# 1mishra/cbc

Hardware: AMD Instinct MI355X
Metric: Mbases/s encoded (bit-exact) on synthetic 150 bp SAM (higher is better)
Workload: dtype u32; 1 GPU; cfg2: synthetic 150 bp SAM, 10000000 reads per GPU vs a 248956422 bp uniform-ACGT contig, block-parallel encode; reads_rank0=10000000, blocks_rank0=2442, block_reads=4096, lds_bytes_per_block=15264, payload_bytes_rank0=20710203, parallelism=one GPU, no collective

## Files before the change

cbc_amd/csrc/cbc_encode_body.h:

```cpp
#ifndef CBC_ENCODE_BODY_H
#define CBC_ENCODE_BODY_H

#include <stdint.h>
#include <type_traits>
#include "../../include/cbc_gpu.h"
#include "cbc_plan.h"

#ifndef CBC_PRIO_CODER
#define CBC_PRIO_CODER 3
#define CBC_PRIO_MODEL 0
#endif
#define CBC_REC_PACK_AT 56u
#define CBC_AWORD     26u
#define CBC_M26       ((1u << 26) - 1u)
#define CBC_M25       ((1u << 25) - 1u)
#define CBC_RESCALE   (1u << 20)
#define CBC_NVARCTX   0xffffu
#define CBC_NOMEMO    0xffffffffu
#define CBC_BLOOM_LOG2 13u
#define CBC_ROLE_FUSED 0u
#define CBC_ROLE_MODEL 1u
#define CBC_ROLE_CODER 2u

#define CBC_LT_MATCH   0u
#define CBC_LT_SAMEREF 8u
#define CBC_LT_CHARS   16u

#define CBC_LDS_RLEN    0u
#define CBC_LDS_SNPS    256u
#define CBC_LDS_INDELS  512u
#define CBC_LDS_RNKEY   768u
#define CBC_LDS_RNEXC   (768u + CBC_CAP_NAME)
#define CBC_LDS_BLOOM   (768u + 2u * CBC_CAP_NAME)
#define CBC_LDS_P0      (768u + 2u * CBC_CAP_NAME + CBC_BLOOM_WORDS)
#define CBC_LDS_BATCH   CBC_PLAN_TABLE_WORDS
#ifndef CBC_BATCH_MIN
#define CBC_BATCH_MIN   40u
#endif
#define CBC_LDS_CTL     (CBC_LDS_BATCH + CBC_BATCH_SLOTS * CBC_BATCH_WORDS)
#define CBC_LDS_RING    (CBC_LDS_CTL + 8u)
#define CBC_LDS_RUN     (CBC_LDS_RING + CBC_RING_WORDS)
#define CBC_LDS_FIXED   CBC_PLAN_LDS_FIXED_WORDS

#ifdef CBC_EMU_TRACE
extern "C" void cbc_emu_trace(uint32_t read, uint32_t lo, uint32_t cnt, uint32_t n);
#endif

struct cbc_enc_args {
    const cbc_read_rec   *recs;
    const uint8_t        *seq;
    const uint32_t       *tok;
    const uint8_t        *names;
    const cbc_block_desc *blocks;
    const uint8_t        *ref;
    uint8_t              *out;
    cbc_block_result     *results;
    uint64_t ref_bytes, out_bytes, seq_bytes, n_tok, n_recs;
    uint32_t n_blocks, cap_pos, cap_var, names_bytes;
};

#if defined(CBC_STAMP) && defined(__HIP_DEVICE_COMPILE__)
#define CBC_T0() do { unsigned long long t_; asm volatile("s_memtime %0\n\ts_waitcnt lgkmcnt(0)" : "=s"(t_) :: "memory"); E.t_last = t_; } while (0)
#define CBC_TS(k) do { unsigned long long t_; asm volatile("s_memtime %0\n\ts_waitcnt lgkmcnt(0)" : "=s"(t_) :: "memory"); E.t_sum[k] += t_ - E.t_last; E.t_last = t_; } while (0)
#define CBC_TSM(k) do { unsigned long long t_; asm volatile("s_memtime %0\n\ts_waitcnt lgkmcnt(0)" : "=s"(t_) :: "memory"); t_sum[k] += t_ - t_last; t_last = t_; } while (0)
#elif defined(CBC_MARKS) && defined(__HIP_DEVICE_COMPILE__)
#define CBC_TSM(k) asm volatile("; ==== CBC_MARK M" #k)
#define CBC_T0() asm volatile("; ==== CBC_MARK start")
#define CBC_TS(k) asm volatile("; ==== CBC_MARK " #k)
#else
#define CBC_T0() do {} while (0)
#define CBC_TS(k) do {} while (0)
#define CBC_TSM(k) do {} while (0)
#endif

CBC_FN bool cbc_le64(uint64_t a, uint64_t b)
{
    uint32_t ah = (uint32_t)(a >> 32), al = (uint32_t)a, bh = (uint32_t)(b >> 32), bl = (uint32_t)b;
    return (ah < bh) | ((ah == bh) & (al <= bl));
}
CBC_FN bool cbc_fits64(uint64_t off, uint64_t len, uint64_t total)
{
    return cbc_le64(off, total) && cbc_le64(len, total - off);
}
CBC_FN uint32_t cbc_avail32(uint64_t total, uint32_t off)
{
    uint64_t a = total - off;
    if (!cbc_le64((uint64_t)off, total)) return 0u;
    return (uint32_t)(a >> 32) ? 0xffffffffu : (uint32_t)a;
}
CBC_FN uint32_t cbc_basepair(uint32_t c)
{
    return c == 'A' ? 0u : c == 'C' ? 1u : c == 'G' ? 2u : c == 'T' ? 3u : 4u;
}
// ... 76 lines not shown
        w2 |= (kw == 2u) ? bit : 0ull;
        w3 |= (kw == 3u) ? bit : 0ull;
    }
#endif
};

template <class W, class = void> struct CbcHasLaneN : std::false_type {};
template <class W> struct CbcHasLaneN<W, std::void_t<decltype(&W::set_lane2_uv), decltype(&W::set_lane3)>> : std::true_type {};

template <class W, bool GEN = false>
struct CbcEnc {
    typedef typename W::V32 V32;
    typedef typename W::Mask Mask;

    typedef typename W::Uv Uv;
    Uv l, rng;
    Uv lm1;
    Uv thr0;
    CBC_MFN void set_l_forms()
    {
        lm1 = W::uv_opaque(l - 1u);
        thr0 = ((l & (1u << 24)) | (1u << 25)) - l;
    }
    uint32_t scale3;
    uint32_t bitpos, flushed;
    uint32_t *ring;
    uint32_t *out32; uint32_t cap_words;
    uint32_t status, nsym, fail_read, cur_read;
    V32 q_lo, q_cnt, q_n; uint32_t q_len;
    uint32_t role, batch_i; uint32_t *batch, *ctl;
    V32 b_lo, b_hi, b_n, b_fl, b_fh; uint32_t b_len, b_pos, b_stop, b_flags, seen_last; uint64_t b_neq;
    V32 rec_a, rec_s; uint32_t rec_n;
#ifdef CBC_STAMP
    unsigned long long t_last, t_sum[16];
#endif

    V32 small;
    V32 fkey, fexc; uint32_t fcount;
    V32 hkey, hexc; uint32_t hc0, hc1, hc2, hc3, hn0, hn1, hn2, hn3;
    uint32_t *rlen_exc, *snps_exc, *indels_exc, *rname_key, *rname_exc, *pos_val, *pos_occ, *pos_pre, *pos_idx, *var_ev, *bloom, *p0ev;
    uint32_t *runs;
    uint32_t snps_n, indels_n;
    uint32_t rn_count, rn_cap;
    uint32_t *vtab;
    uint32_t *fsp_key, *fsp_exc; uint32_t fsp_count;
    uint32_t *pos_ov_val, *pos_ov_occ; uint32_t pos_lds_cap;
    uint32_t *palpha; uint32_t pa_n0, pa_n1, pa_n2, pa_n3;
    uint32_t pos_card, cap_pos;
    uint32_t nev, nev1, cap_var;
    V32 p0cnt; uint32_t p0over;
    uint32_t L0;

    uint32_t prevPos, prevM, prevChar, win_pos;
    CbcWin<W> win;

    CBC_MFN void fail(uint32_t st) { if (status == CBC_ST_OK) { status = st; fail_read = cur_read; } }

    CBC_MFN void place(const V32 &val, const V32 &len, const V32 &off, const Mask &m)
    {
        const V32 aligned = val << (W::splat(32u) - len);
        const V32 sh = off & 31u, w = (off >> 5) & (CBC_RING_WORDS - 1u);
        const Mask on = m & (len != 0u);
        W::lds_or(ring, w, aligned >> sh, on);
        W::lds_or(ring, (w + 1u) & (CBC_RING_WORDS - 1u), aligned << (W::splat(32u) - sh), on & (sh != 0u));
    }
    CBC_MFN void flush_full()
    {
// ... 80 lines not shown
        else {
            V32 ln = W::lane();
            Mask here = ln == q_len;
            q_lo = W::select(here, W::splat(lo), q_lo);
            q_cnt = W::select(here, W::splat(cnt), q_cnt);
            q_n = W::select(here, W::splat(n), q_n);
        }
        q_len++;
    }
    CBC_MFN void rec_put(Uv rec, Uv k3)
    {
        if constexpr (!GEN && CbcHasLaneN<W>::value) W::set_lane2_uv(rec_a, rec_s, rec_n, rec, k3);
        else { W::set_lane_uv(rec_a, rec_n, rec); W::set_lane_uv(rec_s, rec_n, k3); }
    }
#define CBC_FRAC(c, n) W::frac32(c, n)
#define CBC_BF_LAST  1u
#define CBC_BF_GROUP 2u
#define CBC_END_N    0xffffffffu
    CBC_MFN void drain() { if (role == CBC_ROLE_MODEL) publish(0u, 0ull); else drain_q(); }
    CBC_MFN void seg_end()
    {
        if (role != CBC_ROLE_MODEL) { drain_q(); return; }
        if (q_len >= 64u) publish(0u, 0ull);
        q_put(0u, 1u, CBC_END_N);
    }
    CBC_MFN void seg_end_fits()
    {
        W::expect_eq(q_len < 64u ? 1u : 0u, 1u, "seg_end_fits: queue full");
        q_put(0u, 1u, CBC_END_N);
    }
    CBC_MFN void publish(uint32_t flags, uint64_t neq)
    {
        V32 ln = W::lane();
        CBC_TSM(5);
        while (batch_i - W::ctl_load(ctl + 1) >= CBC_BATCH_SLOTS) W::nap();
        CBC_TSM(6);
        uint32_t *buf = batch + (batch_i & (CBC_BATCH_SLOTS - 1u)) * CBC_BATCH_WORDS;
        Mask m = ln < q_len;
        W::store32(buf, ln, q_lo, m); W::store32(buf + 64u, ln, q_cnt, m); W::store32(buf + 128u, ln, q_n, m);
        V32 hdr = W::select(ln == 0u, W::splat(q_len), W::select(ln == 1u, W::splat(flags),
                  W::select(ln == 2u, W::splat(status), W::select(ln == 3u, W::splat(status == CBC_ST_OK ? cur_read : fail_read),
                  W::select(ln == 4u, W::splat((uint32_t)neq), W::splat((uint32_t)(neq >> 32)))))));
        W::store32(buf + 192u, ln, hdr, ln < 6u);
        batch_i++;
        W::ctl_store(ctl, batch_i);
        q_len = 0;
    }
    CBC_MFN void step(uint32_t lo, uint32_t hi, uint32_t n, uint32_t flo, uint32_t fhi)
    {
        Uv rec, k3;
        code1(lo, hi, n, flo, fhi, rec, k3);
        rec_put(rec, k3);
        nsym++;
        if (++rec_n >= CBC_REC_PACK_AT) { pack(rec_a, rec_s, rec_n); rec_n = 0; }
    }
    CBC_MFN void flush_recs() { if (rec_n) { pack(rec_a, rec_s, rec_n); rec_n = 0; } }
    CBC_MFN void room(uint32_t k) { if (rec_n + k >= 64u) flush_recs(); }
    template <class FLO, class FHI, class FN>
    CBC_MFN void step_fixed(FLO lo_of, FHI hi_of, FN n_of, uint32_t flo, uint32_t fhi)
    {
        Uv rec, k3;
        code1_lazy(flo, fhi, lo_of, hi_of, n_of, rec, k3);
#ifdef CBC_ABLATE_SETLANE
        rec_a ^= rec; rec_s ^= k3;
#else
        rec_put(rec, k3);
#endif
        nsym++; rec_n++;
    }
    template <class FLO, class FHI, class FN>
    CBC_MFN void step_fixed_quiet(FLO lo_of, FHI hi_of, FN n_of, uint32_t flo, uint32_t fhi)
    {
#ifdef CBC_ABLATE_CODER
        step_fixed(lo_of, hi_of, n_of, flo, fhi); return;
#endif
        Uv ql, qh, tl, th;
        W::mul64(rng, flo, ql, tl); W::mul64(rng, fhi, qh, th);
        if (W::uv_ge(tl | th, 0xfc000000u)) {
            const uint32_t lo = lo_of(), hi = hi_of(), n = n_of();
            ql += (rng * lo - ql * n >= n) ? 1u : 0u;
// ... 8 lines not shown
        if (W::uv_ge(still & (1u << 25), 1u)) {
#ifndef __HIP_DEVICE_COMPILE__
            const uint32_t lf = W::uv_scalar(l1), uf = W::uv_scalar(u);
            W::expect_eq(W::clz32((((lf ^ uf) & CBC_M26) << 6) | 32u), 0u, "step_fixed_quiet: E1/E2 would shift");
            W::expect_eq(W::clz32(((((~lf | uf) << 7) | 127u))), 0u, "step_fixed_quiet: E3 would shift");
#endif
            l = l1; rng = qh - ql;
            set_l_forms();
            nsym++;
            return;
        }
        Uv rec, k3;
        code_tail(ql, qh, rec, k3);
        rec_put(rec, k3);
        nsym++; rec_n++;
    }
    CBC_MFN void drain_q()
    {
        V32 ln = W::lane();
        uint32_t m = W::uni(q_len);
        const uint64_t bad = W::ballot((ln < m) & ((q_cnt == 0u) | (q_n == 0u)));
        if (bad) m = W::ctz64(bad);
        const V32 q_hi = q_lo + q_cnt;
        const V32 f_lo = CBC_FRAC(q_lo, q_n), f_hi = CBC_FRAC(q_hi, q_n);
        for (uint32_t k = 0; k < m; k++)
            step(W::readlane(q_lo, k), W::readlane(q_hi, k), W::readlane(q_n, k), W::readlane(f_lo, k), W::readlane(f_hi, k));
        if (bad) fail(CBC_ST_ASSERT);
        q_len = 0;
    }
    CBC_MFN void pull()
    {
        V32 ln = W::lane();
        CBC_TSM(9);
        while (W::ctl_load(ctl) == batch_i) W::nap();
        CBC_TSM(10);
        const uint32_t *buf = batch + (batch_i & (CBC_BATCH_SLOTS - 1u)) * CBC_BATCH_WORDS;
        V32 hdr = W::load32(buf + 192u, ln, ln < 6u, 0u);
        const uint32_t len = W::readlane(hdr, 0u);
        const uint32_t pst = W::readlane(hdr, 2u), prec = W::readlane(hdr, 3u);
        b_flags = W::readlane(hdr, 1u);
        b_neq = (uint64_t)W::readlane(hdr, 4u) | ((uint64_t)W::readlane(hdr, 5u) << 32);
        Mask m = ln < len;
        b_lo = W::load32(buf, ln, m, 0u); b_n = W::load32(buf + 128u, ln, m, 1u);
        const V32 cnt = W::load32(buf + 64u, ln, m, 1u);
        b_hi = b_lo + cnt;
        b_fl = CBC_FRAC(b_lo, b_n); b_fh = CBC_FRAC(b_hi, b_n);
        b_len = len > 64u ? 64u : len; b_pos = 0;
        const uint64_t bad = W::ballot(m & ((cnt == 0u) | (b_n == 0u)));
        b_stop = bad ? W::ctz64(bad) : 64u;
        batch_i++;
        W::ctl_store(ctl + 1, batch_i);
        if (b_flags & CBC_BF_LAST) seen_last = 1u;
        if (pst != CBC_ST_OK && status == CBC_ST_OK) { status = pst; fail_read = prec; }
    }
    CBC_MFN void seg_consume()
    {
        const V32 ln = W::lane();
        uint32_t done = 0u;
        while ((done | status) == 0u) {
            if (b_pos == b_len) {
                if (seen_last) fail(CBC_ST_ASSERT);
                else { pull(); if (b_flags & CBC_BF_GROUP) fail(CBC_ST_ASSERT); }
            } else {
                const uint64_t em = W::ballot((b_n == CBC_END_N) & (ln >= b_pos) & (ln < b_len));
                uint32_t kend = em ? W::ctz64(em) : b_len;
                const uint32_t bad = b_stop < kend ? 1u : 0u;
                if (bad) kend = b_stop;
                for (uint32_t k = b_pos; k < kend; k++) {
                    Uv rec, k3;
                    code1_lazy(W::readlane(b_fl, k), W::readlane(b_fh, k), [&]() -> uint32_t { return W::readlane(b_lo, k); },
                               [&]() -> uint32_t { return W::readlane(b_hi, k); }, [&]() -> uint32_t { return W::readlane(b_n, k); }, rec, k3);
                    rec_put(rec, k3);
                    nsym++;
                    if (++rec_n >= CBC_REC_PACK_AT) { pack(rec_a, rec_s, rec_n); rec_n = 0; }
                }
                if (bad) fail(CBC_ST_ASSERT);
                else if (em) { b_pos = kend + 1u; done = 1u; }
                else b_pos = kend;
            }
        }
    }
    CBC_MFN void consume_all()
    {
        while (!seen_last) {
            pull();
            if (status != CBC_ST_OK) continue;
            const uint32_t kend = b_stop < b_len ? b_stop : b_len;
            for (uint32_t k = 0; k < kend; k++) {
                Uv rec, k3;
                code1_lazy(W::readlane(b_fl, k), W::readlane(b_fh, k), [&]() -> uint32_t { return W::readlane(b_lo, k); },
                           [&]() -> uint32_t { return W::readlane(b_hi, k); }, [&]() -> uint32_t { return W::readlane(b_n, k); }, rec, k3);
                rec_put(rec, k3);
                nsym++;
                if (++rec_n >= CBC_REC_PACK_AT) { pack(rec_a, rec_s, rec_n); rec_n = 0; }
            }
            if (b_stop < b_len) fail(CBC_ST_ASSERT);
        }
    }
    CBC_MFN void post_group(uint32_t g, uint64_t neq, uint32_t refused)
    {
        W::write_uni(ctl, 4u + 2u * (g & 1u), (uint32_t)neq);
        W::write_uni(ctl, 5u + 2u * (g & 1u), (uint32_t)(neq >> 32));
        if (refused) W::write_uni(ctl, 3u, 1u);
        W::ctl_store(ctl + 2, g + 1u);
    }
    CBC_MFN void abort_groups()
    {
        W::write_uni(ctl, 3u, 1u);
        W::ctl_store(ctl + 2, 0xffffffffu);
    }
    CBC_MFN bool wait_group(uint32_t g, uint64_t &neq)
    {
        CBC_TSM(5);
        while (W::ctl_load(ctl + 2) < g + 1u) W::nap();
        CBC_TSM(6);
        neq = (uint64_t)W::read_uni(ctl, 4u + 2u * (g & 1u)) | ((uint64_t)W::read_uni(ctl, 5u + 2u * (g & 1u)) << 32);
        return W::read_uni(ctl, 3u) == 0u;
    }
    CBC_MFN uint64_t pull_group()
    {
        if (status != CBC_ST_OK) return 0ull;
        if (b_pos != b_len || seen_last) { fail(CBC_ST_ASSERT); return 0ull; }
        pull();
        if (status == CBC_ST_OK && !(b_flags & CBC_BF_GROUP)) fail(CBC_ST_ASSERT);
        return b_neq;
    }
    CBC_MFN void pull_rest() { while (!seen_last) pull(); }
    CBC_MFN void code1(uint32_t lo, uint32_t hi, uint32_t n, uint32_t flo, uint32_t fhi, Uv &rec, Uv &k3)
    {
        code1_lazy(flo, fhi, [&]() { return lo; }, [&]() { return hi; }, [&]() { return n; }, rec, k3);
    }
    template <class FLO, class FHI, class FN>
    CBC_MFN void code1_lazy(uint32_t flo, uint32_t fhi, FLO lo_of, FHI hi_of, FN n_of, Uv &rec, Uv &k3)
    {
#ifdef CBC_ABLATE_CODER
        l ^= flo; rng ^= fhi; rec = W::uv(0u); k3 = rec; return;
#endif
        const Uv range = rng;
        Uv ql, qh, tl, th;
        W::mul64(range, flo, ql, tl); W::mul64(range, fhi, qh, th);
        if (W::uv_ge(tl | th, 0xfc000000u)) {
            const uint32_t lo = lo_of(), hi = hi_of(), n = n_of();
            ql += (range * lo - ql * n >= n) ? 1u : 0u;
            qh += (range * hi - qh * n >= n) ? 1u : 0u;
        }
#ifndef __HIP_DEVICE_COMPILE__
        W::expect_eq(W::uv_scalar(ql), (uint32_t)((uint64_t)W::uv_scalar(range) * lo_of() / n_of()), "scaled_div(cum)");
        W::expect_eq(W::uv_scalar(qh), (uint32_t)((uint64_t)W::uv_scalar(range) * hi_of() / n_of()), "scaled_div(cum + count)");
#endif
        code_tail(ql, qh, rec, k3);
// ... 865 lines not shown
                }
            }
            CBC_TSM(13);
#undef CBC_SNP
#undef CBC_TOK
#undef CBC_READ_BYTE
    }
};

template <class W, uint32_t ROLE>
CBC_FN void cbc_encode_stream(const cbc_enc_args &A, uint32_t blk, uint32_t *lds)
{
    const uint32_t role = ROLE;
    typedef typename W::V32 V32;
    typedef typename W::Mask Mask;
    const V32 ln = W::lane();
    const cbc_block_desc *bd = A.blocks + blk;
    CbcEnc<W> E;

    const uint64_t rec_base = bd->rec_base, seq_base = bd->seq_base, tok_base = bd->tok_base;
    const uint64_t ref_off = bd->ref_off, out_off = bd->out_off;
    const uint32_t out_cap = bd->out_cap, n_reads = bd->n_reads, name_off = bd->name_off;
    const uint32_t L0 = bd->read_length, n_tok_blk = bd->n_tok;

    E.status = CBC_ST_OK; E.nsym = 0; E.fail_read = 0; E.cur_read = 0;
    E.l = W::uv(0u); E.set_l_forms(); E.rng = W::uv(CBC_M26 + 1u); E.scale3 = 0u; E.bitpos = 0; E.flushed = 0;
    E.ring = lds + CBC_LDS_RING;
    E.q_lo = W::splat(0u); E.q_cnt = W::splat(0u); E.q_n = W::splat(0u); E.q_len = 0;
    E.b_lo = W::splat(0u); E.b_hi = W::splat(0u); E.b_n = W::splat(1u); E.b_fl = W::splat(0u); E.b_fh = W::splat(0u);
    E.b_len = 0; E.b_pos = 0; E.b_stop = 64u; E.b_flags = 0; E.seen_last = 0; E.b_neq = 0;
    E.rec_a = W::splat(0u); E.rec_s = W::splat(0u); E.rec_n = 0;
    E.role = role; E.batch_i = 0; E.batch = lds + CBC_LDS_BATCH; E.ctl = lds + CBC_LDS_CTL;
    if (ROLE != CBC_ROLE_FUSED) {
        if (ROLE == CBC_ROLE_MODEL) { W::write_uni(E.ctl, 0u, 0u); W::write_uni(E.ctl, 1u, 0u); W::write_uni(E.ctl, 2u, 0u); W::write_uni(E.ctl, 3u, 0u); }
        W::barrier();
    }
    const uint32_t payload_cap = bd->reserved;
    E.out32 = (uint32_t *)(A.out + out_off);
    E.cap_words = payload_cap >> 2;
    E.var_ev = (uint32_t *)(A.out + out_off + payload_cap);
    E.cap_var = payload_cap <= out_cap ? (out_cap - payload_cap) >> 2 : 0u;
    bool args_ok = cbc_fits64(out_off, out_cap, A.out_bytes) && ((out_off & 3u) == 0) && ((payload_cap & 3u) == 0) &&
                   (payload_cap <= out_cap) &&
                   cbc_fits64(rec_base, n_reads, A.n_recs) && cbc_fits64(tok_base, n_tok_blk, A.n_tok) &&
                   (L0 >= 1u && L0 <= 256u) && (name_off < A.names_bytes);
    if (!args_ok) { E.cap_words = 0; E.fail(CBC_ST_ASSERT); }
    if (n_reads > CBC_MAX_BLOCK_READS) E.fail(CBC_ST_UNSUPPORTED);

    E.L0 = L0;
    E.rlen_exc = lds + CBC_LDS_RLEN; E.snps_exc = lds + CBC_LDS_SNPS; E.indels_exc = lds + CBC_LDS_INDELS;
    E.rname_key = lds + CBC_LDS_RNKEY; E.rname_exc = lds + CBC_LDS_RNEXC;
    E.bloom = lds + CBC_LDS_BLOOM; E.p0ev = lds + CBC_LDS_P0; E.runs = lds + CBC_LDS_RUN;
    E.pos_val = lds + CBC_LDS_FIXED; E.pos_occ = E.pos_val + A.cap_pos; E.pos_pre = E.pos_occ + A.cap_pos;
    E.fsp_key = E.fsp_exc = nullptr; E.fsp_count = 0; E.pos_ov_val = E.pos_ov_occ = nullptr; E.pos_lds_cap = 0xffffffc0u; E.palpha = nullptr;
    E.pos_idx = E.pos_pre + A.cap_pos;
    E.cap_pos = A.cap_pos;
    if (ROLE != CBC_ROLE_MODEL) {
        for (uint32_t b = 0; b < CBC_POS_IDX_WORDS; b += 64u) W::store32(E.pos_idx, ln + b, W::splat(0u), W::all());
        for (uint32_t b = 0; b < CBC_RING_WORDS; b += 64u) W::store32(E.ring, ln + b, W::splat(0u), W::all());
        for (uint32_t b = 0; b < 256u; b += 64u) W::store32(E.rlen_exc, ln + b, W::splat(0u), W::all());
        W::write_uni(E.pos_val, 0u, 0xffffffffu); W::write_uni(E.pos_occ, 0u, 0u); W::write_uni(E.pos_pre, 0u, 0u);
    }
    if (ROLE != CBC_ROLE_CODER) {
        for (uint32_t b = 0; b < 512u; b += 64u) W::store32(E.snps_exc, ln + b, W::splat(0u), W::all());
        for (uint32_t b = 0; b < CBC_BLOOM_WORDS; b += 64u) W::store32(E.bloom, ln + b, W::splat(0u), W::all());
    }
    E.p0cnt = W::splat(0u); E.p0over = 0;
    E.snps_n = L0; E.indels_n = L0;
    E.rn_count = 0; E.rn_cap = CBC_CAP_NAME; E.vtab = nullptr;
    E.pos_card = 1u;
    E.nev = 0; E.nev1 = 0;
    E.fkey = W::splat(0u); E.fexc = W::splat(0u); E.fcount = 0;
    E.hkey = W::splat(0u); E.hexc = W::splat(0u);
    E.hc0 = E.hc1 = E.hc2 = E.hc3 = 0; E.hn0 = E.hn1 = E.hn2 = E.hn3 = 256u;
    {
        V32 sm = W::splat(0u);
        sm = W::select(ln < 10u, W::splat(1u), sm);
        V32 r = (ln - CBC_LT_CHARS) >> 3, c = (ln - CBC_LT_CHARS) & 7u;
        Mask inch = (ln >= CBC_LT_CHARS) & (r < 6u) & (c < 5u);
        V32 cv = W::select(c == 4u, W::splat(1u), W::select(c == r, W::splat(0u), W::splat(8u)));
        Mask bump = ((r == 0u) & ((c == 1u) | (c == 2u))) | ((r == 1u) & ((c == 0u) | (c == 3u))) |
                    ((r == 2u) & ((c == 0u) | (c == 3u))) | ((r == 3u) & ((c == 1u) | (c == 2u)));
        cv = W::select(bump, cv + 8u, cv);
        sm = W::select(inch, cv, sm);
        E.small = sm;
    }
    E.prevPos = 0; E.prevM = 0; E.prevChar = 0; E.win_pos = 0;
    E.win_clear();

    const uint4 *recs4 = (const uint4 *)(A.recs + rec_base);
    const uint8_t *seqb = A.seq + seq_base;
    const uint32_t *tokb = A.tok + tok_base;
    const uint8_t *refb = A.ref + ref_off;
    const uint64_t seq_avail = cbc_le64(seq_base, A.seq_bytes) ? A.seq_bytes - seq_base : 0;
    const uint64_t ref_avail = cbc_le64(ref_off, A.ref_bytes) ? A.ref_bytes - ref_off : 0;
    const uint32_t seq_lim = cbc_avail32(seq_avail, 0u), ref_lim = cbc_avail32(ref_avail, 0u);
#ifdef CBC_STAMP
    for (int i = 0; i < 16; i++) E.t_sum[i] = 0;
    CBC_T0();
#endif

    auto gen_header = [&]() {
        for (uint32_t k = 0; k < 34u && E.status == CBC_ST_OK; k++) {
            uint32_t v = (k == 0u) ? L0 : (k == 33u) ? 8u : CBC_WELL_SEED;
            E.regsparse_code(E.hkey, E.hexc, 0u, 8u, E.hc0, E.hn0, 256u, 1u, v >> 24, CBC_ST_ASSERT);
            E.regsparse_code(E.hkey, E.hexc, 8u, 8u, E.hc1, E.hn1, 256u, 1u, (v >> 16) & 0xffu, CBC_ST_ASSERT);
            E.regsparse_code(E.hkey, E.hexc, 16u, 8u, E.hc2, E.hn2, 256u, 1u, (v >> 8) & 0xffu, CBC_ST_ASSERT);
            E.regsparse_code(E.hkey, E.hexc, 24u, 8u, E.hc3, E.hn3, 256u, 1u, v & 0xffu, CBC_ST_ASSERT);
            if ((k & 7u) == 7u) E.drain();
        }
    };
    auto gen_rname = [&]() {
        for (uint32_t q = 0; E.status == CBC_ST_OK; q++) {
            uint32_t ch = (name_off + q < A.names_bytes) ? W::read_uni8(A.names, name_off + q) : 0u;
            E.rname_code(E.prevChar, ch);
            if ((q & 31u) == 31u) E.drain();
            if (ch == 0u) break;
            E.prevChar = ch;
        }
    };
    auto gen_sentinel = [&]() {
        if (E.q_len >= 56u) E.drain();
        E.cur_read = n_reads;
        E.rname_code(E.prevChar, (uint32_t)'\n');
        E.rname_code((uint32_t)'\n', 0u);
    };
    auto match_group = [&](uint32_t cn, const V32 &r_pos, const V32 &r_fl, const V32 &r_seq) -> uint64_t {
        const V32 vrl = W::select(ln < cn, r_fl >> 16, W::splat(0u));
        const V32 ro = r_pos - 1u;
        const uint32_t nd = W::uni(W::readlane(W::scan_incl_max(vrl), 63u) >> 2);
        V32 acc = W::splat(0u);
// ... 50 lines not shown
            if (c0 == 0u) { gen_rname(); E.seg_end(); }
            typename CbcEnc<W>::Prep P;
            E.prep_group(P, neq, r_tok, tokb, n_tok_blk);
            CBC_TS(14);
            uint64_t todo = neq;
            V32 nx_seq = W::splat(0u), nx_tok = W::splat(0u);
            uint32_t nx_j = 64u;
            auto prefetch = [&](uint32_t jn) {
                const uint32_t so = W::readlane(r_seq, jn), to = W::readlane(r_tok, jn), nrl = W::readlane(r_fl, jn) >> 16;
                V32 bo = ln * 4u;
                nx_seq = W::load32_bytes(seqb + so, bo, bo < nrl);
                nx_tok = W::load32(tokb + to, ln, (ln + to) < n_tok_blk, 0u);
                nx_j = jn;
            };
            auto prefetch_if_general = [&](uint64_t rest) {
                if (rest) { const uint32_t jn = W::ctz64(rest); if (!((P.ord >> jn) & 1ull)) prefetch(jn); }
            };
            typename CbcEnc<W>::Run R;
            R.pk = W::splat(0u); R.ca = R.pk; R.cb = R.pk; R.rm = 0ull; R.s = 0u; R.counted = 0u;
            while (todo && E.status == CBC_ST_OK) {
                const uint32_t j = W::ctz64(todo);
                if ((P.ord >> j) & 1ull) {
                    if (!E.run_pass(R, P, todo, r_pos, r_fl, r_seq, r_tok, tokb, seqb)) { P.ord &= ~R.rm; continue; }
                    todo &= ~R.rm;
                    prefetch_if_general(todo);
                    CBC_TS(2);
                    for (uint64_t rr = R.rm; rr && E.status == CBC_ST_OK; rr &= rr - 1ull) {
                        const uint32_t jr = W::ctz64(rr);
                        E.cur_read = c0 + jr;
                        E.run_record(R, W::readlane(P.hdr0, jr) >> 16, W::readlane(P.lo, jr), W::readlane(P.cnt, jr));
                        E.seg_end_fits();
                        CBC_TS(1);
                        if (E.q_len >= CBC_BATCH_MIN) E.drain();
                    }
                    continue;
                }
                if (nx_j != j) prefetch(j);
                todo &= todo - 1ull;
                E.cur_read = c0 + j;
                const V32 seqv = nx_seq, tokv = nx_tok;
                prefetch_if_general(todo);
                const typename CbcEnc<W>::PrepRec pr = { W::readlane(P.lo, j), W::readlane(P.cnt, j) };
                E.edits(W::readlane(r_pos, j), W::readlane(r_fl, j), W::readlane(r_tok, j), seqv, tokv, tokb, n_tok_blk, pr);
                E.seg_end_fits();
                CBC_TS(1);
                if (E.q_len >= CBC_BATCH_MIN) E.drain();
            }
        }
        if (E.status == CBC_ST_OK) { gen_sentinel(); E.seg_end(); }
#if defined(CBC_STAMP) && defined(__HIP_DEVICE_COMPILE__)
        if (E.cap_var >= 64u) for (int i = 0; i < 16; i++) {
            W::write_uni(E.var_ev + E.cap_var - 32u, 2 * i, (uint32_t)E.t_sum[i]); W::write_uni(E.var_ev + E.cap_var - 32u, 2 * i + 1, (uint32_t)(E.t_sum[i] >> 32)); }
#endif
        E.publish(CBC_BF_LAST, 0ull);
        return;
    }

    const bool fused = ROLE == CBC_ROLE_FUSED;
    if (!fused) W::prio(CBC_PRIO_CODER);
#ifndef CBC_MATCH_IN_MODEL
    uint64_t neq_ahead = 0;
    auto look_ahead = [&](uint32_t g0) {
        V32 a_pos, a_fl, a_seq, a_tok;
        const uint32_t an = n_reads - g0 < 64u ? n_reads - g0 : 64u;
        const uint32_t saved = E.cur_read;
        CBC_TS(9);
        const bool okg = load_group(g0, a_pos, a_fl, a_seq, a_tok, true);
        neq_ahead = okg ? match_group(an, a_pos, a_fl, a_seq) : 0ull;
        E.post_group(g0 >> 6, neq_ahead, okg ? 0u : 1u);
        CBC_TS(15);
        if (okg) E.cur_read = saved;
    };
    if (!fused && n_reads != 0u && E.status == CBC_ST_OK) look_ahead(0u);
#endif
    if (E.status == CBC_ST_OK) { if (fused) { gen_header(); E.seg_end(); } else E.seg_consume(); }
    for (uint32_t c0 = 0; c0 < n_reads && E.status == CBC_ST_OK; c0 += 64u) {
        V32 r_pos, r_fl, r_seq, r_tok;
        const uint32_t cn = n_reads - c0 < 64u ? n_reads - c0 : 64u;
        E.cur_read = c0;
        uint64_t neq;
        typename CbcEnc<W>::Prep P;
        typename CbcEnc<W>::Run R;
        R.pk = W::splat(0u); R.ca = R.pk; R.cb = R.pk; R.rm = 0ull; R.s = 0u; R.counted = 0u;
        if (fused) {
            if (!load_group(c0, r_pos, r_fl, r_seq, r_tok, true)) break;
            neq = match_group(cn, r_pos, r_fl, r_seq);
// ... 79 lines not shown
        typedef std::integral_constant<int, 0> Plain; typedef std::integral_constant<int, 1> Esc; typedef std::integral_constant<int, 2> Look;
        uint32_t j = 0;
        if (c0 == 0u && jn != 0u) { code_record(0u, std::true_type(), Look()); j = 1u; }
        while (j < jn && E.status == CBC_ST_OK) {
            const uint64_t ahead = F.esc >> j;
            uint32_t run_end = ahead ? j + W::ctz64(ahead) : jn;
            if (run_end > jn) run_end = jn;
            for (; j < run_end && E.status == CBC_ST_OK; j++) code_record(j, std::false_type(), Plain());
            if (j < jn && E.status == CBC_ST_OK) { code_record(j, std::false_type(), Esc()); j++; }
        }
#else
        for (uint32_t j = 0; j < jn && E.status == CBC_ST_OK; j++) code_record(j, 0, std::integral_constant<int, 2>());
#endif
#undef CBC_ENC_FIRST
        if (jn < cn && E.status == CBC_ST_OK) { E.cur_read = c0 + jn; E.fail(W::readlane(F.st, jn)); }
    }
    uint32_t nbytes = 0;
    if (E.status == CBC_ST_OK) {
        E.cur_read = n_reads;
        if (n_reads) E.encode(10u * n_reads - 9u, 11u, 10u * n_reads + 2u);
        else E.encode(1u, 1u, 2u);
        E.drain_q();
        if (fused) { gen_sentinel(); E.seg_end(); } else E.seg_consume();
    }
    if (E.status == CBC_ST_OK) { E.flush_recs(); nbytes = E.finish(); }
    if (E.status != CBC_ST_OK) nbytes = 0;
#ifndef CBC_MATCH_IN_MODEL
#ifndef CBC_MATCH_NO_ABORT_FOR_TEST
    if (!fused && E.status != CBC_ST_OK) E.abort_groups();
#endif
#endif
    if (!fused) E.pull_rest();
#if defined(CBC_STAMP) && defined(__HIP_DEVICE_COMPILE__)
    if (payload_cap >= 128u) for (int i = 0; i < 16; i++) {
        W::write_uni(E.out32, 2 * i, (uint32_t)E.t_sum[i]); W::write_uni(E.out32, 2 * i + 1, (uint32_t)(E.t_sum[i] >> 32)); }
#endif
    V32 resv = W::select(ln == 0u, W::splat(nbytes), W::select(ln == 1u, W::splat(E.status),
               W::select(ln == 2u, W::splat(E.nsym), W::splat(E.fail_read))));
    W::store32((uint32_t *)(A.results + blk), ln, resv, ln < 4u);
}

#endif
```

cbc_amd/csrc/cbc_long_body.h:

```cpp
#ifndef CBC_LONG_BODY_H
#define CBC_LONG_BODY_H

#include "cbc_encode_body.h"
#include "cbc_decode_body.h"

#define CBC_LONG_MAGIC 0x43424C03u
#define CBC_LLDS_GAPLO  0u
#define CBC_LLDS_SP     512u
#define CBC_LLDS_RNKEY  896u
#define CBC_LLDS_RNEXC  (896u + CBC_CAP_NAME)
#define CBC_LLDS_ROLE   (896u + 2u * CBC_CAP_NAME)
#define CBC_LLDS_RING   CBC_LLDS_ROLE
#define CBC_LLDS_BATCH  (CBC_LLDS_ROLE + CBC_RING_WORDS)
#define CBC_LLDS_CTL    (CBC_LLDS_BATCH + CBC_BATCH_SLOTS * CBC_BATCH_WORDS)

#define CBC_LLDS_TRIP   (CBC_LLDS_CTL + 8u)
#define CBC_LLDS_FIXED  (CBC_LLDS_TRIP + 576u)
static inline uint32_t cbc_long_lds_bytes(uint32_t cap_pos) { return 4u * (CBC_LLDS_FIXED + 2u * cap_pos); }
static inline uint32_t cbc_long_dec_lds_bytes(uint32_t cap_pos) { return 4u * (CBC_LLDS_ROLE + 2u * cap_pos); }
#define CBC_LSCR_GAPHI  0u
#define CBC_LSCR_GX     1536u
#define CBC_LSCR_EDITS  2048u
#ifndef CBC_LONG_EDIT_CAP
#define CBC_LONG_EDIT_CAP 8192u
#endif
#define CBC_LONG_EDIT_HALF (CBC_LONG_EDIT_CAP / 2u)
#define CBC_LONG_TABLE_WORDS 2048u
#define CBC_ROLE_WALKER 3u
#define CBC_LONG_SCRATCH_WORDS (2048u + CBC_LONG_EDIT_CAP)

#define CBC_LS_LEN 0u
#define CBC_LS_NE  4u
CBC_FN uint32_t cbc_long_kind_base(uint32_t pk) { return pk < 2u ? pk * 3u : 10u + (pk - 2u) * 3u; }

struct cbc_long_args {
    const cbc_read_rec   *recs;
    const uint8_t        *seq;
    const uint32_t       *tok;
    const uint8_t        *names;
    const cbc_block_desc *blocks;
    const uint8_t        *ref;
    uint8_t              *out;
    cbc_block_result     *results;
    uint64_t ref_bytes, out_bytes, seq_bytes, n_tok, n_recs;
    uint32_t n_blocks, cap_pos, names_bytes;
    uint32_t *scratch;
};
// ... 29 lines not shown
};

template <class W, uint32_t ROLE>
CBC_FN void cbc_long_encode(const cbc_long_args &A, uint32_t blk, uint32_t *lds)
{
    typedef typename W::V32 V32;
    typedef typename W::Mask Mask;
    typedef CbcEnc<W, true> Enc;
    const V32 ln = W::lane();
    const cbc_block_desc *bd = A.blocks + blk;
    Enc E;
    const uint64_t rec_base = bd->rec_base, seq_base = bd->seq_base, tok_base = bd->tok_base, ref_off = bd->ref_off, out_off = bd->out_off;
    const uint32_t out_cap = bd->out_cap, n_reads = bd->n_reads, name_off = bd->name_off, n_tok_blk = bd->n_tok;

    E.status = CBC_ST_OK; E.nsym = 0; E.fail_read = 0; E.cur_read = 0;
    E.l = W::uv(0u); E.set_l_forms(); E.rng = W::uv(CBC_M26 + 1u); E.scale3 = 0u; E.bitpos = 0; E.flushed = 0;
    E.ring = lds + CBC_LLDS_RING;
    E.q_lo = W::splat(0u); E.q_cnt = W::splat(0u); E.q_n = W::splat(0u); E.q_len = 0;
    E.b_lo = W::splat(0u); E.b_hi = W::splat(0u); E.b_n = W::splat(1u); E.b_fl = W::splat(0u); E.b_fh = W::splat(0u);
    E.rec_a = W::splat(0u); E.rec_s = W::splat(0u); E.rec_n = 0;
    E.role = ROLE; E.batch_i = 0; E.batch = lds + CBC_LLDS_BATCH; E.ctl = lds + CBC_LLDS_CTL;
    E.b_len = 0; E.b_pos = 0; E.b_stop = 64u; E.b_flags = 0; E.seen_last = 0; E.b_neq = 0;
    if (ROLE != CBC_ROLE_FUSED) {
        if (ROLE == CBC_ROLE_MODEL) for (uint32_t k = 0; k < 8u; k++) W::write_uni(E.ctl, k, 0u);
        W::barrier();
    }
    E.out32 = (uint32_t *)(A.out + out_off);
    E.cap_words = out_cap >> 2;
    bool args_ok = cbc_fits64(out_off, out_cap, A.out_bytes) && ((out_off & 3u) == 0u) && cbc_fits64(rec_base, n_reads, A.n_recs) &&
                   cbc_fits64(tok_base, n_tok_blk, A.n_tok) && (name_off < A.names_bytes) && A.cap_pos >= 2u && n_reads <= 64u &&
                   A.scratch != nullptr;
    if (!args_ok) { E.cap_words = 0; E.fail(CBC_ST_ASSERT); }
#ifdef CBC_STAMP
    for (int i = 0; i < 16; i++) E.t_sum[i] = 0;
    CBC_T0();
#endif

    if (ROLE == CBC_ROLE_CODER) {
        W::prio(CBC_PRIO_CODER);
        for (uint32_t b = 0; b < CBC_RING_WORDS; b += 64u) W::store32(E.ring, ln + b, W::splat(0u), W::all());
        E.consume_all();
        uint32_t nbytes = 0;
        if (E.status == CBC_ST_OK) { E.flush_recs(); nbytes = E.finish(); }
        if (E.status != CBC_ST_OK) nbytes = 0;
#if defined(CBC_STAMP) && defined(__HIP_DEVICE_COMPILE__)
        CBC_TS(9);
        if (out_cap >= 512u) for (int i = 0; i < 16; i++) {
            W::write_uni(E.out32, 2 * i, (uint32_t)E.t_sum[i]); W::write_uni(E.out32, 2 * i + 1, (uint32_t)(E.t_sum[i] >> 32)); }
#endif
        V32 resv = W::select(ln == 0u, W::splat(nbytes), W::select(ln == 1u, W::splat(E.status),
                   W::select(ln == 2u, W::splat(E.nsym), W::splat(E.fail_read))));
        W::store32((uint32_t *)(A.results + blk), ln, resv, ln < 4u);
        return;
    }

    E.L0 = 256u;
    E.rlen_exc = nullptr; E.snps_exc = nullptr; E.indels_exc = nullptr;
    E.rname_key = lds + CBC_LLDS_RNKEY; E.rname_exc = lds + CBC_LLDS_RNEXC; E.rn_cap = CBC_CAP_NAME; E.rn_count = 0;
    E.pos_val = lds + CBC_LLDS_FIXED; E.pos_occ = E.pos_val + A.cap_pos; E.pos_pre = nullptr; E.cap_pos = A.cap_pos;
    E.fsp_key = E.fsp_exc = nullptr; E.fsp_count = 0; E.pos_ov_val = E.pos_ov_occ = nullptr; E.pos_lds_cap = 0xffffffc0u; E.palpha = nullptr;
    E.bloom = nullptr; E.var_ev = nullptr; E.nev = E.nev1 = 0; E.cap_var = 0; E.vtab = nullptr; E.p0ev = nullptr;
    E.p0cnt = W::splat(0u); E.p0over = 0;
    uint32_t *scr = A.scratch + (uint64_t)blk * CBC_LONG_SCRATCH_WORDS;
    if (ROLE != CBC_ROLE_WALKER) {
        for (uint32_t b = 0; b < CBC_LLDS_SP; b += 64u) W::store32(lds, ln + b, W::splat(0u), W::all());
        if (E.status == CBC_ST_OK) for (uint32_t b = 0; b < CBC_LONG_TABLE_WORDS; b += 64u) W::store32_list(scr, ln + b, W::splat(0u), W::all());
        if (ROLE == CBC_ROLE_FUSED) for (uint32_t b = 0; b < CBC_RING_WORDS; b += 64u) W::store32(E.ring, ln + b, W::splat(0u), W::all());
// ... 740 lines not shown
```

cbc_amd/csrc/cbc_plan.h:

```cpp
#ifndef CBC_PLAN_H
#define CBC_PLAN_H

#include <stdint.h>
#include <string.h>
#include "../../include/cbc_gpu.h"

#define CBC_BLOOM_WORDS 256u
#define CBC_P0_WORDS    512u
#define CBC_P0_BUCKET_WORDS 64u
#define CBC_P0_CAP      128u
#define CBC_PLAN_TABLE_WORDS (768u + 2u * CBC_CAP_NAME + CBC_BLOOM_WORDS + 2u * CBC_P0_WORDS)
#ifndef CBC_BATCH_SLOTS
#define CBC_BATCH_SLOTS 2u
#endif
#define CBC_BATCH_WORDS 200u
#ifndef CBC_POS_IDX_WORDS
#define CBC_POS_IDX_WORDS 256u
#endif
#define CBC_RING_WORDS  256u
#define CBC_RUN_WORDS   16u
#define CBC_PLAN_LDS_FIXED_WORDS (CBC_PLAN_TABLE_WORDS + CBC_BATCH_SLOTS * CBC_BATCH_WORDS + 8u + CBC_RING_WORDS + CBC_RUN_WORDS)

static inline uint32_t cbc_plan_lds_bytes(const cbc_lds_caps *caps)
{
    return 4u * (CBC_PLAN_LDS_FIXED_WORDS + 3u * caps->cap_pos + CBC_POS_IDX_WORDS);
}

#define CBC_PLAN_DLDS_SCRATCH_WORDS 336u
#define CBC_PLAN_DLDS_FIXED_WORDS (CBC_PLAN_TABLE_WORDS + CBC_PLAN_DLDS_SCRATCH_WORDS + 768u)
static inline uint32_t cbc_plan_dec_lds_bytes(const cbc_lds_caps *caps)
{
    return 4u * (CBC_PLAN_DLDS_FIXED_WORDS + 2u * caps->cap_pos);
}

static inline uint64_t cbc_plan_block_area(cbc_block_desc *bd, uint64_t off, uint64_t nev)
{
    const uint64_t nsym = 136u + 2u * CBC_CAP_NAME + 16ull * bd->n_reads + 2 * nev;
    uint64_t payload_cap = (3 * nsym + 256 + 255) & ~255ull;
    uint64_t cap = payload_cap + ((4 * (nev + 64) + 255) & ~255ull);
    if (cap > 0xffffff00ull) { cap = 0xffffff00ull; payload_cap = cap / 2; payload_cap &= ~255ull; }
    bd->out_off = off; bd->out_cap = (uint32_t)cap; bd->reserved = (uint32_t)payload_cap;
    return cap;
}

static inline uint64_t cbc_plan_output(cbc_block_desc *blocks, uint32_t n_blocks,
                                       const cbc_read_rec *recs, const uint32_t *tok)
{
    uint64_t off = 0;
    for (uint32_t b = 0; b < n_blocks; b++) {
        cbc_block_desc *bd = &blocks[b];
        uint64_t nev = 0;
        for (uint32_t r = 0; r < bd->n_reads; r++) {
            const cbc_read_rec *rr = &recs[bd->rec_base + r];
            const uint32_t *t = tok + bd->tok_base + rr->tok_off;
// ... 75 lines not shown
```

Before: 235,300 Mbases/s.

## Parameterize model-coder hand-off ring and add acked multi-slot group masks

```diff
diff --git a/cbc_amd/csrc/cbc_encode_body.h b/cbc_amd/csrc/cbc_encode_body.h
--- a/cbc_amd/csrc/cbc_encode_body.h
+++ b/cbc_amd/csrc/cbc_encode_body.h
@@ -35,10 +35,16 @@
 #define CBC_LDS_P0      (768u + 2u * CBC_CAP_NAME + CBC_BLOOM_WORDS)
 #define CBC_LDS_BATCH   CBC_PLAN_TABLE_WORDS
 #ifndef CBC_BATCH_MIN
-#define CBC_BATCH_MIN   40u
-#endif
-#define CBC_LDS_CTL     (CBC_LDS_BATCH + CBC_BATCH_SLOTS * CBC_BATCH_WORDS)
-#define CBC_LDS_RING    (CBC_LDS_CTL + 8u)
+#define CBC_BATCH_MIN   (5u * CBC_BATCH_ENTRIES / 8u)
+#endif
+#define CBC_LDS_CTL     (CBC_LDS_BATCH + CBC_BATCH_SLOTS * CBC_BATCH_SLOT_WORDS)
+#define CBC_LDS_RING    (CBC_LDS_CTL + CBC_CTL_WORDS)
+#define CBC_CTL_PRODUCED 0u
+#define CBC_CTL_CONSUMED 1u
+#define CBC_CTL_POSTED   2u
+#define CBC_CTL_REFUSED  3u
+#define CBC_CTL_ACKED    4u
+#define CBC_CTL_MASKS    5u
 #define CBC_LDS_RUN     (CBC_LDS_RING + CBC_RING_WORDS)
 #define CBC_LDS_FIXED   CBC_PLAN_LDS_FIXED_WORDS
 
@@ -59,6 +65,7 @@
     uint32_t n_blocks, cap_pos, cap_var, names_bytes;
 };
 
+#define CBC_STAMP_SLOTS 20
 #if defined(CBC_STAMP) && defined(__HIP_DEVICE_COMPILE__)
 #define CBC_T0() do { unsigned long long t_; asm volatile("s_memtime %0\n\ts_waitcnt lgkmcnt(0)" : "=s"(t_) :: "memory"); E.t_last = t_; } while (0)
 #define CBC_TS(k) do { unsigned long long t_; asm volatile("s_memtime %0\n\ts_waitcnt lgkmcnt(0)" : "=s"(t_) :: "memory"); E.t_sum[k] += t_ - E.t_last; E.t_last = t_; } while (0)
@@ -201,7 +208,7 @@
     V32 b_lo, b_hi, b_n, b_fl, b_fh; uint32_t b_len, b_pos, b_stop, b_flags, seen_last; uint64_t b_neq;
     V32 rec_a, rec_s; uint32_t rec_n;
 #ifdef CBC_STAMP
-    unsigned long long t_last, t_sum[16];
+    unsigned long long t_last, t_sum[CBC_STAMP_SLOTS];
 #endif
 
     V32 small;
@@ -348,20 +355,54 @@
     CBC_MFN void publish(uint32_t flags, uint64_t neq)
     {
         V32 ln = W::lane();
-        CBC_TSM(5);
-        while (batch_i - W::ctl_load(ctl + 1) >= CBC_BATCH_SLOTS) W::nap();
-        CBC_TSM(6);
-        uint32_t *buf = batch + (batch_i & (CBC_BATCH_SLOTS - 1u)) * CBC_BATCH_WORDS;
-        Mask m = ln < q_len;
-        W::store32(buf, ln, q_lo, m); W::store32(buf + 64u, ln, q_cnt, m); W::store32(buf + 128u, ln, q_n, m);
-        V32 hdr = W::select(ln == 0u, W::splat(q_len), W::select(ln == 1u, W::splat(flags),
-                  W::select(ln == 2u, W::splat(status), W::select(ln == 3u, W::splat(status == CBC_ST_OK ? cur_read : fail_read),
-                  W::select(ln == 4u, W::splat((uint32_t)neq), W::splat((uint32_t)(neq >> 32)))))));
-        W::store32(buf + 192u, ln, hdr, ln < 6u);
-        batch_i++;
-        W::ctl_store(ctl, batch_i);
-        q_len = 0;
-    }
+        if constexpr (GEN) {
+            CBC_TSM(5);
+#ifdef CBC_STAMP
+            t_sum[18] += 1u; if (batch_i - W::ctl_load(ctl + 1) >= CBC_LONG_BATCH_SLOTS) t_sum[17] += 1u;
+#endif
+            while (batch_i - W::ctl_load(ctl + 1) >= CBC_LONG_BATCH_SLOTS) W::nap();
+            CBC_TSM(6);
+            uint32_t *buf = batch + (batch_i & (CBC_LONG_BATCH_SLOTS - 1u)) * CBC_LONG_BATCH_WORDS;
+            Mask m = ln < q_len;
+            W::store32(buf, ln, q_lo, m); W::store32(buf + 64u, ln, q_cnt, m); W::store32(buf + 128u, ln, q_n, m);
+            V32 hdr = W::select(ln == 0u, W::splat(q_len), W::select(ln == 1u, W::splat(flags),
+                      W::select(ln == 2u, W::splat(status), W::select(ln == 3u, W::splat(status == CBC_ST_OK ? cur_read : fail_read),
+                      W::select(ln == 4u, W::splat((uint32_t)neq), W::splat((uint32_t)(neq >> 32)))))));
+            W::store32(buf + 192u, ln, hdr, ln < 6u);
+            batch_i++;
+            W::ctl_store(ctl, batch_i);
+            q_len = 0;
+        } else {
+            uint32_t off = 0u;
+            do {
+                const uint32_t left = q_len - off;
+                const uint32_t n = CBC_BATCH_ENTRIES >= 64u || left < CBC_BATCH_ENTRIES ? left : CBC_BATCH_ENTRIES;
+                const uint32_t fl = n == left ? flags : 0u;
+                CBC_TSM(5);
+#ifdef CBC_STAMP
+                t_sum[18] += 1u; if (batch_i - W::ctl_load(ctl + CBC_CTL_CONSUMED) >= CBC_BATCH_SLOTS) t_sum[17] += 1u;
+#endif
+                while (batch_i - W::ctl_load(ctl + CBC_CTL_CONSUMED) >= CBC_BATCH_SLOTS) W::nap();
+                CBC_TSM(6);
+                uint32_t *buf = batch + (batch_i % CBC_BATCH_SLOTS) * CBC_BATCH_SLOT_WORDS;
+                const V32 k = ln - off;
+                const Mask m = k < n;
+                W::store32(buf, k, q_lo, m); W::store32(buf + CBC_BATCH_ENTRIES, k, q_cnt, m); W::store32(buf + 2u * CBC_BATCH_ENTRIES, k, q_n, m);
+#ifdef CBC_MATCH_IN_MODEL
+                if (fl & CBC_BF_GROUP) { W::write_uni(buf, 0u, (uint32_t)neq); W::write_uni(buf, 1u, (uint32_t)(neq >> 32)); }
+#endif
+                const V32 hdr = W::select(ln == 0u, W::splat(n | (fl << 8) | (status << 16)), W::splat(status == CBC_ST_OK ? cur_read : fail_read));
+                W::store32(buf + 3u * CBC_BATCH_ENTRIES, ln, hdr, ln < 2u);
+                batch_i++;
+                W::ctl_store(ctl + CBC_CTL_PRODUCED, batch_i);
+                off += n;
+            } while (CBC_BATCH_ENTRIES < 64u && off < q_len);
+            q_len = 0;
+        }
+    }
+#ifdef CBC_HANDOFF_ADAPTIVE
+    CBC_MFN bool coder_near() { return batch_i - W::ctl_load(ctl + CBC_CTL_CONSUMED) <= 1u; }
+#endif
     CBC_MFN void step(uint32_t lo, uint32_t hi, uint32_t n, uint32_t flo, uint32_t fhi)
     {
         Uv rec, k3;
@@ -436,26 +477,52 @@
     {
         V32 ln = W::lane();
         CBC_TSM(9);
+#ifdef CBC_STAMP
+        t_sum[18] += 1u; if (W::ctl_load(ctl) == batch_i) t_sum[17] += 1u;
+#endif
         while (W::ctl_load(ctl) == batch_i) W::nap();
         CBC_TSM(10);
-        const uint32_t *buf = batch + (batch_i & (CBC_BATCH_SLOTS - 1u)) * CBC_BATCH_WORDS;
-        V32 hdr = W::load32(buf + 192u, ln, ln < 6u, 0u);
-        const uint32_t len = W::readlane(hdr, 0u);
-        const uint32_t pst = W::readlane(hdr, 2u), prec = W::readlane(hdr, 3u);
-        b_flags = W::readlane(hdr, 1u);
-        b_neq = (uint64_t)W::readlane(hdr, 4u) | ((uint64_t)W::readlane(hdr, 5u) << 32);
-        Mask m = ln < len;
-        b_lo = W::load32(buf, ln, m, 0u); b_n = W::load32(buf + 128u, ln, m, 1u);
-        const V32 cnt = W::load32(buf + 64u, ln, m, 1u);
-        b_hi = b_lo + cnt;
-        b_fl = CBC_FRAC(b_lo, b_n); b_fh = CBC_FRAC(b_hi, b_n);
-        b_len = len > 64u ? 64u : len; b_pos = 0;
-        const uint64_t bad = W::ballot(m & ((cnt == 0u) | (b_n == 0u)));
-        b_stop = bad ? W::ctz64(bad) : 64u;
-        batch_i++;
-        W::ctl_store(ctl + 1, batch_i);
-        if (b_flags & CBC_BF_LAST) seen_last = 1u;
-        if (pst != CBC_ST_OK && status == CBC_ST_OK) { status = pst; fail_read = prec; }
+        if constexpr (GEN) {
+            const uint32_t *buf = batch + (batch_i & (CBC_LONG_BATCH_SLOTS - 1u)) * CBC_LONG_BATCH_WORDS;
+            V32 hdr = W::load32(buf + 192u, ln, ln < 6u, 0u);
+            const uint32_t len = W::readlane(hdr, 0u);
+            const uint32_t pst = W::readlane(hdr, 2u), prec = W::readlane(hdr, 3u);
+            b_flags = W::readlane(hdr, 1u);
+            b_neq = (uint64_t)W::readlane(hdr, 4u) | ((uint64_t)W::readlane(hdr, 5u) << 32);
+            Mask m = ln < len;
+            b_lo = W::load32(buf, ln, m, 0u); b_n = W::load32(buf + 128u, ln, m, 1u);
+            const V32 cnt = W::load32(buf + 64u, ln, m, 1u);
+            b_hi = b_lo + cnt;
+            b_fl = CBC_FRAC(b_lo, b_n); b_fh = CBC_FRAC(b_hi, b_n);
+            b_len = len > 64u ? 64u : len; b_pos = 0;
+            const uint64_t bad = W::ballot(m & ((cnt == 0u) | (b_n == 0u)));
+            b_stop = bad ? W::ctz64(bad) : 64u;
+            batch_i++;
+            W::ctl_store(ctl + 1, batch_i);
+            if (b_flags & CBC_BF_LAST) seen_last = 1u;
+            if (pst != CBC_ST_OK && status == CBC_ST_OK) { status = pst; fail_read = prec; }
+        } else {
+            const uint32_t *buf = batch + (batch_i % CBC_BATCH_SLOTS) * CBC_BATCH_SLOT_WORDS;
+            const V32 hdrv = W::load32(buf + 3u * CBC_BATCH_ENTRIES, ln, ln < 2u, 0u);
+            const uint32_t hdr = W::readlane(hdrv, 0u), prec = W::readlane(hdrv, 1u);
+            const uint32_t len = hdr & 0xffu, pst = hdr >> 16;
+            b_flags = (hdr >> 8) & 0xffu;
+            Mask m = ln < len;
+            b_lo = W::load32(buf, ln, m, 0u); b_n = W::load32(buf + 2u * CBC_BATCH_ENTRIES, ln, m, 1u);
+            const V32 cnt = W::load32(buf + CBC_BATCH_ENTRIES, ln, m, 1u);
+#ifdef CBC_MATCH_IN_MODEL
+            if (b_flags & CBC_BF_GROUP) b_neq = (uint64_t)W::read_uni(buf, 0u) | ((uint64_t)W::read_uni(buf, 1u) << 32);
+#endif
+            b_hi = b_lo + cnt;
+            b_fl = CBC_FRAC(b_lo, b_n); b_fh = CBC_FRAC(b_hi, b_n);
+            b_len = len > CBC_BATCH_ENTRIES ? CBC_BATCH_ENTRIES : len; b_pos = 0;
+            const uint64_t bad = W::ballot(m & ((cnt == 0u) | (b_n == 0u)));
+            b_stop = bad ? W::ctz64(bad) : 64u;
+            batch_i++;
+            W::ctl_store(ctl + CBC_CTL_CONSUMED, batch_i);
+            if (b_flags & CBC_BF_LAST) seen_last = 1u;
+            if (pst != CBC_ST_OK && status == CBC_ST_OK) { status = pst; fail_read = prec; }
+        }
     }
     CBC_MFN void seg_consume()
     {
@@ -503,23 +570,26 @@
     }
     CBC_MFN void post_group(uint32_t g, uint64_t neq, uint32_t refused)
     {
-        W::write_uni(ctl, 4u + 2u * (g & 1u), (uint32_t)neq);
-        W::write_uni(ctl, 5u + 2u * (g & 1u), (uint32_t)(neq >> 32));
-        if (refused) W::write_uni(ctl, 3u, 1u);
-        W::ctl_store(ctl + 2, g + 1u);
+        while (g >= CBC_MASK_SLOTS && W::ctl_load(ctl + CBC_CTL_ACKED) < g - (CBC_MASK_SLOTS - 1u)) W::nap();
+        W::write_uni(ctl, CBC_CTL_MASKS + 2u * (g % CBC_MASK_SLOTS), (uint32_t)neq);
+        W::write_uni(ctl, CBC_CTL_MASKS + 1u + 2u * (g % CBC_MASK_SLOTS), (uint32_t)(neq >> 32));
+        if (refused) W::write_uni(ctl, CBC_CTL_REFUSED, 1u);
+        W::ctl_store(ctl + CBC_CTL_POSTED, g + 1u);
     }
     CBC_MFN void abort_groups()
     {
-        W::write_uni(ctl, 3u, 1u);
-        W::ctl_store(ctl + 2, 0xffffffffu);
+        W::write_uni(ctl, CBC_CTL_REFUSED, 1u);
+        W::ctl_store(ctl + CBC_CTL_POSTED, 0xffffffffu);
     }
     CBC_MFN bool wait_group(uint32_t g, uint64_t &neq)
     {
         CBC_TSM(5);
-        while (W::ctl_load(ctl + 2) < g + 1u) W::nap();
-        CBC_TSM(6);
-        neq = (uint64_t)W::read_uni(ctl, 4u + 2u * (g & 1u)) | ((uint64_t)W::read_uni(ctl, 5u + 2u * (g & 1u)) << 32);
-        return W::read_uni(ctl, 3u) == 0u;
+        while (W::ctl_load(ctl + CBC_CTL_POSTED) < g + 1u) W::nap();
+        CBC_TSM(16);
+        neq = (uint64_t)W::read_uni(ctl, CBC_CTL_MASKS + 2u * (g % CBC_MASK_SLOTS)) | ((uint64_t)W::read_uni(ctl, CBC_CTL_MASKS + 1u + 2u * (g % CBC_MASK_SLOTS)) << 32);
+        const bool ok = W::read_uni(ctl, CBC_CTL_REFUSED) == 0u;
+        W::ctl_store(ctl + CBC_CTL_ACKED, g + 1u);
+        return ok;
     }
     CBC_MFN uint64_t pull_group()
     {
@@ -1451,7 +1521,7 @@
     E.rec_a = W::splat(0u); E.rec_s = W::splat(0u); E.rec_n = 0;
     E.role = role; E.batch_i = 0; E.batch = lds + CBC_LDS_BATCH; E.ctl = lds + CBC_LDS_CTL;
     if (ROLE != CBC_ROLE_FUSED) {
-        if (ROLE == CBC_ROLE_MODEL) { W::write_uni(E.ctl, 0u, 0u); W::write_uni(E.ctl, 1u, 0u); W::write_uni(E.ctl, 2u, 0u); W::write_uni(E.ctl, 3u, 0u); }
+        if (ROLE == CBC_ROLE_MODEL) for (uint32_t k = 0; k < CBC_CTL_MASKS; k++) W::write_uni(E.ctl, k, 0u);
         W::barrier();
     }
     const uint32_t payload_cap = bd->reserved;
@@ -1515,7 +1585,7 @@
     const uint64_t ref_avail = cbc_le64(ref_off, A.ref_bytes) ? A.ref_bytes - ref_off : 0;
     const uint32_t seq_lim = cbc_avail32(seq_avail, 0u), ref_lim = cbc_avail32(ref_avail, 0u);
 #ifdef CBC_STAMP
-    for (int i = 0; i < 16; i++) E.t_sum[i] = 0;
+    for (int i = 0; i < CBC_STAMP_SLOTS; i++) E.t_sum[i] = 0;
     CBC_T0();
 #endif
 
@@ -1632,6 +1702,9 @@
                         E.seg_end_fits();
                         CBC_TS(1);
                         if (E.q_len >= CBC_BATCH_MIN) E.drain();
+#ifdef CBC_HANDOFF_ADAPTIVE
+                        else if (E.coder_near()) E.drain();
+#endif
                     }
                     continue;
                 }
@@ -1645,13 +1718,17 @@
                 E.seg_end_fits();
                 CBC_TS(1);
                 if (E.q_len >= CBC_BATCH_MIN) E.drain();
+#ifdef CBC_HANDOFF_ADAPTIVE
+                else if (E.coder_near()) E.drain();
+#endif
             }
         }
         if (E.status == CBC_ST_OK) { gen_sentinel(); E.seg_end(); }
 #if defined(CBC_STAMP) && defined(__HIP_DEVICE_COMPILE__)
-        if (E.cap_var >= 64u) for (int i = 0; i < 16; i++) {
-            W::write_uni(E.var_ev + E.cap_var - 32u, 2 * i, (uint32_t)E.t_sum[i]); W::write_uni(E.var_ev + E.cap_var - 32u, 2 * i + 1, (uint32_t)(E.t_sum[i] >> 32)); }
-#endif
+        if (E.cap_var >= 64u) for (int i = 0; i < CBC_STAMP_SLOTS; i++) {
+            W::write_uni(E.var_ev + E.cap_var - 2u * CBC_STAMP_SLOTS, 2 * i, (uint32_t)E.t_sum[i]); W::write_uni(E.var_ev + E.cap_var - 2u * CBC_STAMP_SLOTS, 2 * i + 1, (uint32_t)(E.t_sum[i] >> 32)); }
+#endif
+        W::ctl_store(E.ctl + CBC_CTL_ACKED, 0xffffffffu);
         E.publish(CBC_BF_LAST, 0ull);
         return;
     }
@@ -1797,7 +1874,7 @@
 #endif
     if (!fused) E.pull_rest();
 #if defined(CBC_STAMP) && defined(__HIP_DEVICE_COMPILE__)
-    if (payload_cap >= 128u) for (int i = 0; i < 16; i++) {
+    if (payload_cap >= 8u * CBC_STAMP_SLOTS) for (int i = 0; i < CBC_STAMP_SLOTS; i++) {
         W::write_uni(E.out32, 2 * i, (uint32_t)E.t_sum[i]); W::write_uni(E.out32, 2 * i + 1, (uint32_t)(E.t_sum[i] >> 32)); }
 #endif
     V32 resv = W::select(ln == 0u, W::splat(nbytes), W::select(ln == 1u, W::splat(E.status),
diff --git a/cbc_amd/csrc/cbc_long_body.h b/cbc_amd/csrc/cbc_long_body.h
--- a/cbc_amd/csrc/cbc_long_body.h
+++ b/cbc_amd/csrc/cbc_long_body.h
@@ -12,7 +12,7 @@
 #define CBC_LLDS_ROLE   (896u + 2u * CBC_CAP_NAME)
 #define CBC_LLDS_RING   CBC_LLDS_ROLE
 #define CBC_LLDS_BATCH  (CBC_LLDS_ROLE + CBC_RING_WORDS)
-#define CBC_LLDS_CTL    (CBC_LLDS_BATCH + CBC_BATCH_SLOTS * CBC_BATCH_WORDS)
+#define CBC_LLDS_CTL    (CBC_LLDS_BATCH + CBC_LONG_BATCH_SLOTS * CBC_LONG_BATCH_WORDS)
 
 #define CBC_LLDS_TRIP   (CBC_LLDS_CTL + 8u)
 #define CBC_LLDS_FIXED  (CBC_LLDS_TRIP + 576u)
@@ -108,7 +108,7 @@
                    A.scratch != nullptr;
     if (!args_ok) { E.cap_words = 0; E.fail(CBC_ST_ASSERT); }
 #ifdef CBC_STAMP
-    for (int i = 0; i < 16; i++) E.t_sum[i] = 0;
+    for (int i = 0; i < CBC_STAMP_SLOTS; i++) E.t_sum[i] = 0;
     CBC_T0();
 #endif
 
diff --git a/cbc_amd/csrc/cbc_plan.h b/cbc_amd/csrc/cbc_plan.h
--- a/cbc_amd/csrc/cbc_plan.h
+++ b/cbc_amd/csrc/cbc_plan.h
@@ -13,13 +13,27 @@
 #ifndef CBC_BATCH_SLOTS
 #define CBC_BATCH_SLOTS 2u
 #endif
-#define CBC_BATCH_WORDS 200u
+#ifndef CBC_BATCH_ENTRIES
+#define CBC_BATCH_ENTRIES 64u
+#endif
+#define CBC_BATCH_SLOT_WORDS (3u * CBC_BATCH_ENTRIES + 2u)
+#define CBC_MASK_SLOTS 4u
+#define CBC_CTL_WORDS (5u + 2u * CBC_MASK_SLOTS)
+#define CBC_HANDOFF_WORDS (CBC_BATCH_SLOTS * CBC_BATCH_SLOT_WORDS + CBC_CTL_WORDS)
+#if CBC_BATCH_ENTRIES > 64u || CBC_BATCH_ENTRIES < 8u || CBC_BATCH_SLOTS < 2u
+#error "hand-off ring: 8..64 entries per slot, >= 2 slots"
+#endif
+#if CBC_HANDOFF_WORDS > 408u && !defined(CBC_HANDOFF_OVER_LDS)
+#error "hand-off ring and control words exceed 408 LDS words"
+#endif
+#define CBC_LONG_BATCH_SLOTS 2u
+#define CBC_LONG_BATCH_WORDS 200u
 #ifndef CBC_POS_IDX_WORDS
 #define CBC_POS_IDX_WORDS 256u
 #endif
 #define CBC_RING_WORDS  256u
 #define CBC_RUN_WORDS   16u
-#define CBC_PLAN_LDS_FIXED_WORDS (CBC_PLAN_TABLE_WORDS + CBC_BATCH_SLOTS * CBC_BATCH_WORDS + 8u + CBC_RING_WORDS + CBC_RUN_WORDS)
+#define CBC_PLAN_LDS_FIXED_WORDS (CBC_PLAN_TABLE_WORDS + CBC_HANDOFF_WORDS + CBC_RING_WORDS + CBC_RUN_WORDS)
 
 static inline uint32_t cbc_plan_lds_bytes(const cbc_lds_caps *caps)
 {
```

Result: no change. 235,700 Mbases/s, median of 3 (+0.1%).
